# RuntimeRacer/vall-e

Hardware: AMD Instinct MI355X
Metric: AR codec-tokens/sec/GPU + NAR 7-stage p50 latency, d=1024 L=12 10s utterance (higher is better)
Workload: dtype bf16

## Files before the change

### vall-e_amd/csrc/ar_tp.hpp

```cpp
#pragma once
#include <type_traits>
#include "ar_granules.hpp"

namespace vx {

#ifdef VX_STAMPS
#define TP_STAMP(which, i)                                                                                            \
  do {                                                                                                                \
    unsigned long long* fq_r_ = g_fq_stamps;                                                                          \
    if (fq_r_ != nullptr && threadIdx.x == 0)                                                                         \
      fq_r_[(((size_t)(which) * 16 + a.layer) * 256 + blockIdx.x) * 16 + (i)] = __builtin_amdgcn_s_memrealtime();      \
  } while (0)
#else
#define TP_STAMP(which, i) do { } while (0)
#endif

constexpr int TP_D = 1024, TP_H = 16, TP_FF = 4096, TP_X = 8, TP_WG = 32;
constexpr int TP_HID = TP_FF / TP_X;
constexpr int TP_ACH = TP_D / TP_X;

struct TpAccArgs {
  long long* add;
  long long* zero;
  const float* bias;
};
constexpr float TP_FIX = 4294967296.0f, TP_UNFIX = 2.3283064365386963e-10f;
__device__ __forceinline__ long long tp_fix(float v) { return __float2ll_rn(v * TP_FIX); }

struct TpAttnArgs {
  const float* qkv_bias;
  unsigned* err;
  fq_gran* gq;
  fq_gran* gp;
  TpAccArgs acc;
  void* kcache;
  void* vcache;
  int ctx_max;
  float scale;
  int layer;
};

struct TpFfnArgs {
  const float* b1;
  unsigned* err;
  fq_gran* gh;
  TpAccArgs acc;
  int layer;
};

struct TpHeadArgs {
  float* logits;
  int N;
};

typedef float tp_f4 __attribute__((ext_vector_type(4)));
__device__ __forceinline__ void tp_ld16(vx_u32x4& v, const void* p) {
  asm volatile("global_load_dwordx4 %0, %1, off" : "=v"(v) : "v"(p) : "memory");
}
__device__ __forceinline__ void tp_ld16w(vx_u32x4& v, const void* p) {
  asm volatile("global_load_dwordx4 %0, %1, off" : "=v"(v) : "v"(p) : "memory");
}
__device__ __forceinline__ void tp_ld16f(tp_f4& v, const void* p) {
  asm volatile("global_load_dwordx4 %0, %1, off" : "=v"(v) : "v"(p) : "memory");
}
__device__ __forceinline__ void tp_ld4f(float& v, const void* p) {
  asm volatile("global_load_dword %0, %1, off" : "=v"(v) : "v"(p) : "memory");
}
template <int N> __device__ __forceinline__ void tp_wait() { asm volatile("s_waitcnt vmcnt(%0)" ::"n"(N) : "memory"); }
template <int N> __device__ __forceinline__ void tp_wait(vx_u32x4& a) { asm volatile("s_waitcnt vmcnt(%1)" : "+v"(a) : "n"(N) : "memory"); }
template <int N> __device__ __forceinline__ void tp_wait(float& a) { asm volatile("s_waitcnt vmcnt(%1)" : "+v"(a) : "n"(N) : "memory"); }
__device__ __forceinline__ uint4 tp_u4(const vx_u32x4& v) { return make_uint4(v.x, v.y, v.z, v.w); }

struct TpRowLoads { tp_f4 x, g, be; vx_u32x4 xf[2]; };
template <bool FIRST>
__device__ __forceinline__ void tp_row_issue(TpRowLoads& r, const float* __restrict__ x_f32, const long long* __restrict__ racc,
                                             const float* __restrict__ gbb, int tid) {
  if (FIRST) {
    tp_ld16f(r.x, x_f32 + 4 * tid);
  } else {
    tp_ld16(r.xf[0], racc + 4 * tid);
    tp_ld16(r.xf[1], racc + 4 * tid + 2);
  }
  tp_ld16f(r.g, gbb + 4 * tid);
  tp_ld16f(r.be, gbb + TP_D + 4 * tid);
}
template <bool FIRST, int AFTER> __device__ __forceinline__ void tp_row_wait(TpRowLoads& r) {
  if (FIRST) asm volatile("s_waitcnt vmcnt(%3)" : "+v"(r.x), "+v"(r.g), "+v"(r.be) : "n"(AFTER) : "memory");
  else asm volatile("s_waitcnt vmcnt(%4)" : "+v"(r.xf[0]), "+v"(r.xf[1]), "+v"(r.g), "+v"(r.be) : "n"(AFTER) : "memory");
}
__device__ __forceinline__ float tp_unfix(unsigned lo, unsigned hi) {
  return __ll2float_rn((long long)(((unsigned long long)hi << 32) | lo)) * TP_UNFIX;
}
template <typename WT> __device__ __forceinline__ float tp_exp(float v) {
  if constexpr (std::is_same<WT, float>::value) return expf(v);
  else return __expf(v);
}
template <bool FIRST>
__device__ __forceinline__ void tp_row_norm(TpRowLoads& r, float* xs, float* red, int tid) {
  const int lane = tid & 63, wave = tid >> 6;
  float4 v;
  if (FIRST) v = make_float4(r.x.x, r.x.y, r.x.z, r.x.w);
  else v = make_float4(tp_unfix(r.xf[0].x, r.xf[0].y), tp_unfix(r.xf[0].z, r.xf[0].w), tp_unfix(r.xf[1].x, r.xf[1].y), tp_unfix(r.xf[1].z, r.xf[1].w));
  float s1 = wave_sum_dpp((v.x + v.y) + (v.z + v.w));
  if (lane == 0) red[wave] = s1;
  __syncthreads();
  const float mean = ((red[0] + red[1]) + (red[2] + red[3])) * (1.0f / TP_D);
  const float d0 = v.x - mean, d1 = v.y - mean, d2 = v.z - mean, d3 = v.w - mean;
  float s2 = wave_sum_dpp((d0 * d0 + d1 * d1) + (d2 * d2 + d3 * d3));
  if (lane == 0) red[4 + wave] = s2;
  __syncthreads();
  const float rstd = 1.0f / sqrtf(((red[4] + red[5]) + (red[6] + red[7])) * (1.0f / TP_D) + LN_EPS);
  *reinterpret_cast<float4*>(xs + 4 * tid) =
      make_float4(d0 * rstd * r.g.x + r.be.x, d1 * rstd * r.g.y + r.be.y, d2 * rstd * r.g.z + r.be.z, d3 * rstd * r.g.w + r.be.w);
  __syncthreads();
}

template <bool FIRST>
__device__ __forceinline__ void tp_acc_add(const TpAccArgs& a, float partial, bool writer, int row, bool lead,
                                           unsigned long long carry_ll, float carry_f, float bo) {
  if (writer) {
    long long add = tp_fix(partial);
    if (lead) add += tp_fix(bo) + (FIRST ? tp_fix(carry_f) : (long long)carry_ll);
    atomicAdd(reinterpret_cast<unsigned long long*>(a.add) + row, (unsigned long long)add);
  }
}
__device__ __forceinline__ void tp_acc_zero(const TpAccArgs& a, bool zeroer, int tid) {
  if (zeroer) {
    *reinterpret_cast<uint4*>(a.zero + 4 * tid) = make_uint4(0u, 0u, 0u, 0u);
    *reinterpret_cast<uint4*>(a.zero + 4 * tid + 2) = make_uint4(0u, 0u, 0u, 0u);
  }
}
template <bool FIRST>
__device__ __forceinline__ void tp_acc_tail(const TpAccArgs& a, float partial, bool writer, int row, bool lead, int tid,
                                            unsigned long long carry_ll, float carry_f, float bo) {
  tp_acc_add<FIRST>(a, partial, writer, row, lead, carry_ll, carry_f, bo);
  tp_acc_zero(a, blockIdx.x == 1, tid);
}

template <int KCH, int VEC>
__device__ __forceinline__ void tp_row_read(const float* xs, int lane, float (&xr)[KCH][VEC]) {
#pragma unroll
  for (int c = 0; c < KCH; ++c)
#pragma unroll
    for (int i = 0; i < VEC; i += 4) {
      const float4 t = *reinterpret_cast<const float4*>(xs + (c * 64 + lane) * VEC + i);
      xr[c][i] = t.x; xr[c][i + 1] = t.y; xr[c][i + 2] = t.z; xr[c][i + 3] = t.w;
    }
}
template <typename WT, int KCH>
__device__ __forceinline__ float tp_dot(const uint4 (&w)[KCH], const float (&xr)[KCH][Vec16<WT>::N]) {
  constexpr int VEC = Vec16<WT>::N;
  float s = 0.f;
#pragma unroll
  for (int c = 0; c < KCH; ++c) {
    float wf[VEC];
    unpack<WT>(w[c], wf);
#pragma unroll
    for (int i = 0; i < VEC; ++i) s = fmaf(wf[i], xr[c][i], s);
  }
  return s;
}

template <int NGRP> struct TpAttnSmem {
  __attribute__((aligned(16))) float xs[TP_D];
  float red[8];
  __attribute__((aligned(16))) float s_qkv[FQ_QKV];
  __attribute__((aligned(16))) float sm_o[NGRP][64 + 4];
  float sm_m[4], sm_l[4];
  float s_wo[4][64];
  float s_part[FQ_S * FQ_PART];
  float s_fac[FQ_S];
  __attribute__((aligned(16))) float s_att[64];
};

template <typename WT, bool FIRST>
__device__ __forceinline__ void tp_attn_split(const void* __restrict__ Wqkv_, const float* __restrict__ x_f32,
                                              const long long* __restrict__ racc, const float* __restrict__ gbb,
                                              const ArState* __restrict__ st, const unsigned* __restrict__ epoch,
                                              const TpAttnArgs& a, TpAttnSmem<4 * Vec16<WT>::N>& sm) {
  constexpr int VEC = Vec16<WT>::N;
  constexpr int KCH = TP_D / (64 * VEC);
  constexpr int HD = 64;
  constexpr int LPK = HD / VEC, KPW = 64 / LPK, KPB = 4 * KPW, UNR = 4;
  float* const xs = sm.xs;
  float* const s_qkv = sm.s_qkv;
  const int tid = threadIdx.x, lane = tid & 63, wave = tid >> 6;
  const int x = blockIdx.x & (TP_X - 1), i = blockIdx.x >> 3;
  const int hl = i >> 4, j = i & 15, h = 2 * x + hl;
  const int cih = 8 * j + 2 * wave, ch = h * HD + cih;
  const int st_row = st->row;
  const unsigned tag = *epoch;
  const WT* __restrict__ W = reinterpret_cast<const WT*>(Wqkv_);

  TpRowLoads rl;
  tp_row_issue<FIRST>(rl, x_f32, racc, gbb, tid);
  TP_STAMP(0, 0);
  vx_u32x4 w[2][KCH];
#pragma unroll
  for (int r = 0; r < 2; ++r)
#pragma unroll
    for (int c = 0; c < KCH; ++c) tp_ld16w(w[r][c], W + (size_t)(ch + r) * TP_D + (c * 64 + lane) * VEC);
  float e_bias;
  {
    const float* bp = a.qkv_bias;
    asm volatile("" : "+s"(bp));
    tp_ld4f(e_bias, bp + ch + min(lane, 1));
  }
  const int n_old = st_row;
  const int chunk = (n_old + FQ_S - 1) / FQ_S;
  const int j0 = j * chunk, j1 = min(n_old, j0 + chunk);
  const int sub = lane % LPK, grp = lane / LPK;
  vx_u32x4 kr[UNR], vr[UNR];
  const WT* kb;
  const WT* vb;
  {
    const void* kcp = a.kcache;
    const void* vcp = a.vcache;
    int ctxm = a.ctx_max;
    asm volatile("" : "+s"(kcp), "+s"(vcp), "+s"(ctxm));
    kb = reinterpret_cast<const WT*>(kcp) + (size_t)h * ctxm * HD + sub * VEC;
    vb = reinterpret_cast<const WT*>(vcp) + (size_t)h * ctxm * HD + sub * VEC;
#pragma unroll
    for (int u = 0; u < UNR; ++u) {
      const int jk = min(j0 + u * KPB + wave * KPW + grp, max(j1, 1) - 1);
      tp_ld16(kr[u], kb + (size_t)jk * HD);
      tp_ld16(vr[u], vb + (size_t)jk * HD);
    }
  }
  auto load_pass = [&](int base) {
#pragma unroll
    for (int u = 0; u < UNR; ++u) {
      const int jk = min(base + u * KPB + wave * KPW + grp, max(j1, 1) - 1);
      const uint4 k4 = ld16(kb + (size_t)jk * HD), v4 = ld16(vb + (size_t)jk * HD);
      kr[u] = vx_u32x4{k4.x, k4.y, k4.z, k4.w};
      vr[u] = vx_u32x4{v4.x, v4.y, v4.z, v4.w};
    }
  };
  constexpr int N_KV = 2 * UNR, N_W = 2 * KCH;

  tp_row_wait<FIRST, N_W + 1 + N_KV>(rl);
  TP_STAMP(0, 7);
  tp_row_norm<FIRST>(rl, xs, sm.red, tid);
  TP_STAMP(0, 1);
  {
    float xr[KCH][VEC];
    tp_row_read<KCH, VEC>(xs, lane, xr);
    float acc[2];
#pragma unroll
    for (int r = 0; r < 2; ++r) {
      uint4 wr[KCH];
#pragma unroll
      for (int c = 0; c < KCH; ++c) { tp_wait<N_KV + 1>(w[r][c]); wr[c] = tp_u4(w[r][c]); }
      acc[r] = wave_sum_dpp(tp_dot<WT, KCH>(wr, xr));
    }
    tp_wait<N_KV>(e_bias);
    if (lane < 2) gran_store(a.gq + (size_t)h * FQ_QKV + cih + lane, (lane == 0 ? acc[0] : acc[1]) + e_bias, tag);
  }
  TP_STAMP(0, 2);
  const bool own_wg = (j == FQ_S - 1);
  {
    const int ng = own_wg ? FQ_QKV : HD;
    float v1[1];
    gran_gather<1>(a.gq + (size_t)h * FQ_QKV, ng, tag, v1, a.err, 1u);
    if (tid < ng) s_qkv[tid] = v1[0];
  }
#pragma unroll
  for (int u = 0; u < UNR; ++u) { tp_wait<0>(kr[u]); tp_wait<0>(vr[u]); }
  TP_STAMP(0, 3);
  __syncthreads();
  TP_STAMP(0, 8);
  float qv[VEC];
#pragma unroll
  for (int c = 0; c < VEC; ++c) qv[c] = s_qkv[sub * VEC + c] * a.scale;

  float M = -INFINITY, L = 0.f, acc[VEC];
#pragma unroll
  for (int c = 0; c < VEC; ++c) acc[c] = 0.f;
  const bool owner = own_wg && wave == 0;
  float sn = -INFINITY;
  if (owner) {
    float dot = 0.f;
#pragma unroll
    for (int c = 0; c < VEC; ++c) dot = fmaf(s_qkv[HD + sub * VEC + c], qv[c], dot);
    sn = (LPK == 8) ? group8_sum_dpp(dot) : group16_sum_dpp(dot);
  }
  for (int base = j0; base < j1 || (owner && base == j0); base += UNR * KPB) {
    if (base != j0) load_pass(base);
    const int nr = (j1 - base + KPB - 1) / KPB;
    float sc[UNR], mloc = (base == j0) ? sn : -INFINITY;
#pragma unroll
    for (int u = 0; u < UNR; ++u) {
      sc[u] = -INFINITY;
      if (u < nr) {
        const int jk = base + u * KPB + wave * KPW + grp;
        float kf[VEC];
        unpack<WT>(tp_u4(kr[u]), kf);
        float dot = 0.f;
#pragma unroll
        for (int c = 0; c < VEC; ++c) dot = fmaf(kf[c], qv[c], dot);
        dot = (LPK == 8) ? group8_sum_dpp(dot) : group16_sum_dpp(dot);
        sc[u] = (jk < j1) ? dot : -INFINITY;
        mloc = fmaxf(mloc, sc[u]);
      }
    }
    mloc = wave_max_dpp(mloc);
    if (mloc != -INFINITY) {
      const float Mn = fmaxf(M, mloc);
      const float corr = (M == -INFINITY) ? 0.f : tp_exp<WT>(M - Mn);
      L *= corr;
#pragma unroll
      for (int c = 0; c < VEC; ++c) acc[c] *= corr;
      M = Mn;
#pragma unroll
      for (int u = 0; u < UNR; ++u)
        if (u < nr) {
          float vf[VEC];
          unpack<WT>(tp_u4(vr[u]), vf);
          const float p = tp_exp<WT>(sc[u] - M);
          L += p;
#pragma unroll
          for (int c = 0; c < VEC; ++c) acc[c] = fmaf(p, vf[c], acc[c]);
        }
      if (owner && base == j0 && grp == 0) {
        const float p = tp_exp<WT>(sn - M);
        L += p;
#pragma unroll
        for (int c = 0; c < VEC; ++c) acc[c] = fmaf(p, s_qkv[2 * HD + sub * VEC + c], acc[c]);
      }
    }
  }
  TP_STAMP(0, 9);
  {
#pragma unroll
    for (int c = 0; c < VEC; c += 4)
      *reinterpret_cast<float4*>(&sm.sm_o[wave * KPW + grp][sub * VEC + c]) = make_float4(acc[c], acc[c + 1], acc[c + 2], acc[c + 3]);
    __builtin_amdgcn_fence(__ATOMIC_RELEASE, "wavefront");
    __builtin_amdgcn_wave_barrier();
    float oc = 0.f;
#pragma unroll
    for (int g = 0; g < KPW; ++g) oc += sm.sm_o[wave * KPW + g][lane];
    const float Lw = wave_sum_dpp(sub == 0 ? L : 0.f);
    sm.s_wo[wave][lane] = oc;
    if (lane == 0) { sm.sm_m[wave] = M; sm.sm_l[wave] = Lw; }
  }
  TP_STAMP(0, 10);
  __syncthreads();
  TP_STAMP(0, 11);
  if (tid < FQ_PART) {
    const float Mx = fmaxf(fmaxf(sm.sm_m[0], sm.sm_m[1]), fmaxf(sm.sm_m[2], sm.sm_m[3]));
    float v = 0.f;
    if (tid == HD) {
      v = Mx;
    } else {
#pragma unroll
      for (int wv = 0; wv < 4; ++wv)
        v = fmaf(tid < HD ? sm.s_wo[wv][tid] : sm.sm_l[wv], (sm.sm_m[wv] == -INFINITY) ? 0.f : tp_exp<WT>(sm.sm_m[wv] - Mx), v);
    }
    gran_store(a.gp + ((size_t)h * FQ_S + j) * FQ_PART + tid, v, tag);
  }
  TP_STAMP(0, 4);
  TP_STAMP(0, 5); TP_STAMP(0, 6);
}

template <typename WT, bool FIRST>
__device__ __forceinline__ void tp_attn_proj(const void* __restrict__ Wqkv_, const float* __restrict__ x_f32,
                                             const long long* __restrict__ racc, const float* __restrict__ gbb,
                                             const ArState* __restrict__ st, const unsigned* __restrict__ epoch,
                                             const void* __restrict__ Wo_, const TpAttnArgs& a,
                                             TpAttnSmem<4 * Vec16<WT>::N>& sm) {
  constexpr int VEC = Vec16<WT>::N;
  constexpr int KCH = TP_D / (64 * VEC);
  constexpr int HD = 64;
  constexpr int OCH = HD / (4 * VEC);
  float* const xs = sm.xs;
  const int tid = threadIdx.x, lane = tid & 63, wave = tid >> 6;
  const int x = blockIdx.x & (TP_X - 1), i = blockIdx.x >> 3;
  const int hl = i >> 4, jp = (i & 15) - FQ_S, h = 2 * x + hl;
  const int cih = 8 * jp + 2 * wave, ch = h * HD + cih;
  const int st_row = st->row, st_done = st->done;
  const unsigned tag = *epoch;
  const WT* __restrict__ W = reinterpret_cast<const WT*>(Wqkv_);

  TpRowLoads rl;
  tp_row_issue<FIRST>(rl, x_f32, racc, gbb, tid);
  TP_STAMP(0, 0);
  vx_u32x4 w[4][KCH];
#pragma unroll
  for (int r = 0; r < 4; ++r)
#pragma unroll
    for (int c = 0; c < KCH; ++c)
      tp_ld16w(w[r][c], W + (size_t)((1 + (r >> 1)) * TP_D + ch + (r & 1)) * TP_D + (c * 64 + lane) * VEC);
  float e_bias;
  {
    const float* bp = a.qkv_bias;
    asm volatile("" : "+s"(bp));
    const int r = min(lane, 3);
    tp_ld4f(e_bias, bp + (1 + (r >> 1)) * TP_D + ch + (r & 1));
  }
  const int orow = 128 * jp + (tid >> 2);
  unsigned long long carry_ll[2] = {0ull, 0ull};
  float carry_f[2] = {0.f, 0.f}, bo[2];
#pragma unroll
  for (int s = 0; s < 2; ++s) {
    if (FIRST) tp_ld4f(carry_f[s], x_f32 + orow + 64 * s);
    else asm volatile("global_load_dwordx2 %0, %1, off" : "=v"(carry_ll[s]) : "v"(racc + orow + 64 * s) : "memory");
    tp_ld4f(bo[s], a.acc.bias + orow + 64 * s);
  }
  vx_u32x4 wo[2][OCH];
  {
    const uint4* wb = reinterpret_cast<const uint4*>(Wo_) + (size_t)(x * TP_WG + 16 * hl + 2 * jp) * OCH * 256;
#pragma unroll
    for (int s = 0; s < 2; ++s)
#pragma unroll
      for (int m = 0; m < OCH; ++m) tp_ld16w(wo[s][m], wb + (s * OCH + m) * 256 + tid);
  }
  constexpr int N_WO = 2 * OCH, N_W = 4 * KCH;

  tp_row_wait<FIRST, N_W + 5 + N_WO>(rl);
  TP_STAMP(0, 7);
  tp_row_norm<FIRST>(rl, xs, sm.red, tid);
  TP_STAMP(0, 1);
  {
    float xr[KCH][VEC];
    tp_row_read<KCH, VEC>(xs, lane, xr);
    float acc[4];
#pragma unroll
    for (int r = 0; r < 4; ++r) {
      uint4 wr[KCH];
#pragma unroll
      for (int c = 0; c < KCH; ++c) { tp_wait<N_WO + 5>(w[r][c]); wr[c] = tp_u4(w[r][c]); }
      acc[r] = wave_sum_dpp(tp_dot<WT, KCH>(wr, xr));
    }
    tp_wait<N_WO + 4>(e_bias);
    if (lane < 4) {
      const int kv = lane >> 1, c = cih + (lane & 1);
      const WT rv = from_f32<WT>((lane == 0 ? acc[0] : lane == 1 ? acc[1] : lane == 2 ? acc[2] : acc[3]) + e_bias);
      if (!st_done) {
        WT* cache = reinterpret_cast<WT*>(kv == 0 ? a.kcache : a.vcache);
        cache[((size_t)h * a.ctx_max + st_row) * HD + c] = rv;
      }
      gran_store(a.gq + (size_t)h * FQ_QKV + (1 + kv) * HD + c, to_f32(rv), tag);
    }
  }
  TP_STAMP(0, 2);
  TP_STAMP(0, 3); TP_STAMP(0, 8); TP_STAMP(0, 9); TP_STAMP(0, 10); TP_STAMP(0, 11); TP_STAMP(0, 4);
  {
    constexpr int NG = (FQ_S * FQ_PART + 255) / 256;
    float pv[NG];
    gran_gather<NG>(a.gp + (size_t)h * FQ_S * FQ_PART, FQ_S * FQ_PART, tag, pv, a.err, 2u);
#pragma unroll
    for (int g = 0; g < NG; ++g)
      if (tid + 256 * g < FQ_S * FQ_PART) sm.s_part[tid + 256 * g] = pv[g];
  }
#pragma unroll
  for (int s = 0; s < 2; ++s) {
#pragma unroll
    for (int m = 0; m < OCH; ++m) tp_wait<0>(wo[s][m]);
    asm volatile("" : "+v"(carry_ll[s]), "+v"(carry_f[s]), "+v"(bo[s]));
  }
  TP_STAMP(0, 5);
  __syncthreads();
  if (tid < FQ_S) {
    const float* hp = sm.s_part;
    float Mx = hp[HD];
#pragma unroll
    for (int s = 1; s < FQ_S; ++s) Mx = fmaxf(Mx, hp[s * FQ_PART + HD]);
    const float pm = hp[tid * FQ_PART + HD];
    const float es = (pm == -INFINITY) ? 0.f : tp_exp<WT>(pm - Mx);
    const float Ls = group8_sum_dpp(hp[tid * FQ_PART + HD + 1] * es);
    sm.s_fac[tid] = es * (1.0f / Ls);
  }
  __syncthreads();
  if (tid < HD) {
    float o = 0.f;
#pragma unroll
    for (int s = 0; s < FQ_S; ++s) o = fmaf(sm.s_part[s * FQ_PART + tid], sm.s_fac[s], o);
    sm.s_att[tid] = o;
  }
  __syncthreads();
#pragma unroll
  for (int sl = 0; sl < 2; ++sl) {
    float s = 0.f;
#pragma unroll
    for (int m = 0; m < OCH; ++m) {
      float wf[VEC];
      unpack<WT>(tp_u4(wo[sl][m]), wf);
      const float* ap = sm.s_att + ((tid & 3) + 4 * m) * VEC;
#pragma unroll
      for (int c = 0; c < VEC; ++c) s = fmaf(wf[c], ap[c], s);
    }
    s = group4_sum_dpp(s);
    tp_acc_add<FIRST>(a.acc, s, (tid & 3) == 0, orow + 64 * sl, h == 0, carry_ll[sl], carry_f[sl], bo[sl]);
  }
  tp_acc_zero(a.acc, blockIdx.x == TP_X * FQ_S + 1, tid);
  TP_STAMP(0, 6);
}

template <typename WT, bool FIRST>
__global__ __launch_bounds__(256) void tp_attn_kernel(const void* __restrict__ Wqkv_, const float* __restrict__ x_f32,
                                                      const long long* __restrict__ racc, const float* __restrict__ gbb,
                                                      const ArState* __restrict__ st, const unsigned* __restrict__ epoch,
                                                      const void* __restrict__ Wo_, const TpAttnArgs a) {
  __shared__ TpAttnSmem<4 * Vec16<WT>::N> sm;
  if (((blockIdx.x >> 3) & (FQ_G - 1)) < FQ_S) tp_attn_split<WT, FIRST>(Wqkv_, x_f32, racc, gbb, st, epoch, a, sm);
  else tp_attn_proj<WT, FIRST>(Wqkv_, x_f32, racc, gbb, st, epoch, Wo_, a, sm);
}

template <typename WT>
__global__ __launch_bounds__(256) void tp_ffn_kernel(const void* __restrict__ W1_, const long long* __restrict__ racc,
                                                     const float* __restrict__ gbb,
                                                     const unsigned* __restrict__ epoch, const void* __restrict__ W2_,
                                                     const TpFfnArgs a) {
  constexpr int VEC = Vec16<WT>::N;
  constexpr int KCH = TP_D / (64 * VEC);
  constexpr int FCH = TP_HID / (8 * VEC);
  __shared__ __attribute__((aligned(16))) float xs[TP_D];
  __shared__ float red[8];
  __shared__ __attribute__((aligned(16))) float hs[TP_HID];
  const int tid = threadIdx.x, lane = tid & 63, wave = tid >> 6;
  const int x = blockIdx.x & (TP_X - 1), i = blockIdx.x >> 3;
  const unsigned tag = *epoch;
  const WT* __restrict__ W1 = reinterpret_cast<const WT*>(W1_);
  const int row0 = TP_HID * x + 16 * i + 4 * wave;

  TpRowLoads rl;
  tp_row_issue<false>(rl, nullptr, racc, gbb, tid);
  TP_STAMP(1, 0);
  vx_u32x4 w1[4][KCH];
#pragma unroll
  for (int r = 0; r < 4; ++r)
#pragma unroll
    for (int c = 0; c < KCH; ++c) tp_ld16w(w1[r][c], W1 + (size_t)(row0 + r) * TP_D + (c * 64 + lane) * VEC);
  float e_b1;
  {
    const float* bp = a.b1;
    asm volatile("" : "+s"(bp));
    tp_ld4f(e_b1, bp + row0 + min(lane, 3));
  }
  unsigned long long carry_ll;
  float bo;
  asm volatile("global_load_dwordx2 %0, %1, off" : "=v"(carry_ll) : "v"(racc + 32 * i + (tid >> 3)) : "memory");
  tp_ld4f(bo, a.acc.bias + 32 * i + (tid >> 3));
  vx_u32x4 w2[FCH];
  auto tp_stage2 = [&]() {
    const uint4* wb = reinterpret_cast<const uint4*>(W2_) + (size_t)(x * TP_WG + i) * FCH * 256;
#pragma unroll
    for (int m = 0; m < FCH; ++m) tp_ld16w(w2[m], wb + m * 256 + tid);
  };
  tp_stage2();
  tp_row_wait<false, 4 * KCH + 3 + FCH>(rl);
  TP_STAMP(1, 7);
  tp_row_norm<false>(rl, xs, red, tid);
  TP_STAMP(1, 1);
  {
    float xr[KCH][VEC];
    tp_row_read<KCH, VEC>(xs, lane, xr);
    float acc[4];
#pragma unroll
    for (int r = 0; r < 4; ++r) {
      uint4 wr[KCH];
#pragma unroll
      for (int c = 0; c < KCH; ++c) { tp_wait<3 + FCH>(w1[r][c]); wr[c] = tp_u4(w1[r][c]); }
      acc[r] = wave_sum_dpp(tp_dot<WT, KCH>(wr, xr));
    }
    tp_wait<2 + FCH>(e_b1);
    if (lane < 4) {
      const float v = (lane == 0 ? acc[0] : lane == 1 ? acc[1] : lane == 2 ? acc[2] : acc[3]) + e_b1;
      gran_store(a.gh + (size_t)x * TP_HID + 16 * i + 4 * wave + lane, fmaxf(v, 0.f), tag);
    }
  }
  TP_STAMP(1, 2);
  {
    float hv[2];
    gran_gather<2>(a.gh + (size_t)x * TP_HID, TP_HID, tag, hv, a.err, 3u);
    hs[tid] = hv[0]; hs[tid + 256] = hv[1];
  }
#pragma unroll
  for (int m = 0; m < FCH; ++m) tp_wait<0>(w2[m]);
  asm volatile("" : "+v"(carry_ll), "+v"(bo));
  TP_STAMP(1, 3);
  __syncthreads();
  {
    float s = 0.f;
#pragma unroll
    for (int m = 0; m < FCH; ++m) {
      float wf[VEC];
      unpack<WT>(tp_u4(w2[m]), wf);
      const float* hp = hs + ((tid & 7) + 8 * m) * VEC;
#pragma unroll
      for (int c = 0; c < VEC; ++c) s = fmaf(wf[c], hp[c], s);
    }
    s = group8_sum_dpp(s);
    tp_acc_tail<false>(a.acc, s, (tid & 7) == 0, 32 * i + (tid >> 3), x == 0, tid, carry_ll, 0.f, bo);
  }
  TP_STAMP(1, 4);
}

template <typename WT>
__global__ __launch_bounds__(256) void tp_head_kernel(const void* __restrict__ W_, const long long* __restrict__ racc,
                                                      const float* __restrict__ gbb,
                                                      const ArState* __restrict__ st, const TpHeadArgs a) {
  constexpr int VEC = Vec16<WT>::N;
  constexpr int KCH = TP_D / (64 * VEC);
  __shared__ __attribute__((aligned(16))) float xs[TP_D];
  __shared__ float red[8];
  const int tid = threadIdx.x, lane = tid & 63, wave = tid >> 6;
  const WT* __restrict__ W = reinterpret_cast<const WT*>(W_);
  const int row0 = (blockIdx.x * 4 + wave) * 4;
  TpRowLoads rl;
  tp_row_issue<false>(rl, nullptr, racc, gbb, tid);
  vx_u32x4 w[4][KCH];
#pragma unroll
  for (int r = 0; r < 4; ++r)
#pragma unroll
    for (int c = 0; c < KCH; ++c) tp_ld16w(w[r][c], W + (size_t)min(row0 + r, a.N - 1) * TP_D + (c * 64 + lane) * VEC);
  const int st_pass = st->pass, st_trace = st->trace_logits, st_done = st->done;
  tp_row_wait<false, 4 * KCH>(rl);
  tp_row_norm<false>(rl, xs, red, tid);
  float xr[KCH][VEC];
  tp_row_read<KCH, VEC>(xs, lane, xr);
  float acc[4];
#pragma unroll
  for (int r = 0; r < 4; ++r) {
    uint4 wr[KCH];
#pragma unroll
    for (int c = 0; c < KCH; ++c) { tp_wait<0>(w[r][c]); wr[c] = tp_u4(w[r][c]); }
    acc[r] = wave_sum_dpp(tp_dot<WT, KCH>(wr, xr));
  }
  const int row = row0 + lane;
  if (lane < 4 && row < a.N && !st_done) {
    const float v = lane == 0 ? acc[0] : lane == 1 ? acc[1] : lane == 2 ? acc[2] : acc[3];
    a.logits[row] = v;
    if (st_trace) a.logits[LOGITS_CUR + (size_t)st_pass * a.N + row] = v;
  }
}

template <typename WT, bool HEADS>
__global__ void tp_repack_kernel(const WT* __restrict__ src, uint4* __restrict__ dst, int K) {
  constexpr int VEC = Vec16<WT>::N;
  const int KX = K / TP_X, NW = KX / (8 * VEC);
  const size_t word = (size_t)blockIdx.x * 256 + threadIdx.x;
  const size_t total = (size_t)TP_D * K / VEC;
  if (word >= total) return;
  const int t = (int)(word & 255);
  const size_t blk = word >> 8;
  const int m = (int)(blk % NW);
  const int wg = (int)(blk / NW);
  const int x = wg / TP_WG, i = wg % TP_WG;
  int row, col;
  if (HEADS) {
    row = 64 * (i & 15) + (t >> 2);
    col = 64 * (2 * x + (i >> 4)) + ((t & 3) + 4 * m) * VEC;
  } else {
    row = 32 * i + (t >> 3);
    col = KX * x + ((t & 7) + 8 * m) * VEC;
  }
  dst[word] = *reinterpret_cast<const uint4*>(src + (size_t)row * K + col);
}

}
```

Measured before the change: 5124.

## Move current-token attention score from split workgroup into the output-projection merge stage

The split-attention stage no longer has one designated workgroup per head that waits for the full new q/k/v row and folds the current token's score and value into its partial softmax. Instead, the merge/output-projection stage gathers the new q/k/v, computes the self-score there, and adds it as an extra term in the cross-split softmax combine. This removes the extra wait and imbalance on the owner workgroup in the attention pass. In exchange it adds a gather and a barrier to the merge stage, which now has to wait for the freshly written K/V before it can finish.

New measurement: 5148, median of 2. Within noise of the previous version (+0.5%).

```diff
diff --git a/vall-e_amd/csrc/ar_tp.hpp b/vall-e_amd/csrc/ar_tp.hpp
--- a/vall-e_amd/csrc/ar_tp.hpp
+++ b/vall-e_amd/csrc/ar_tp.hpp
@@ -169,7 +169,7 @@
   float sm_m[4], sm_l[4];
   float s_wo[4][64];
   float s_part[FQ_S * FQ_PART];
-  float s_fac[FQ_S];
+  float s_fac[FQ_S + 1];
   __attribute__((aligned(16))) float s_att[64];
 };
 
@@ -257,12 +257,10 @@
     if (lane < 2) gran_store(a.gq + (size_t)h * FQ_QKV + cih + lane, (lane == 0 ? acc[0] : acc[1]) + e_bias, tag);
   }
   TP_STAMP(0, 2);
-  const bool own_wg = (j == FQ_S - 1);
-  {
-    const int ng = own_wg ? FQ_QKV : HD;
+  {
     float v1[1];
-    gran_gather<1>(a.gq + (size_t)h * FQ_QKV, ng, tag, v1, a.err, 1u);
-    if (tid < ng) s_qkv[tid] = v1[0];
+    gran_gather<1>(a.gq + (size_t)h * FQ_QKV, HD, tag, v1, a.err, 1u);
+    if (tid < HD) s_qkv[tid] = v1[0];
   }
 #pragma unroll
   for (int u = 0; u < UNR; ++u) { tp_wait<0>(kr[u]); tp_wait<0>(vr[u]); }
@@ -276,18 +274,10 @@
   float M = -INFINITY, L = 0.f, acc[VEC];
 #pragma unroll
   for (int c = 0; c < VEC; ++c) acc[c] = 0.f;
-  const bool owner = own_wg && wave == 0;
-  float sn = -INFINITY;
-  if (owner) {
-    float dot = 0.f;
-#pragma unroll
-    for (int c = 0; c < VEC; ++c) dot = fmaf(s_qkv[HD + sub * VEC + c], qv[c], dot);
-    sn = (LPK == 8) ? group8_sum_dpp(dot) : group16_sum_dpp(dot);
-  }
-  for (int base = j0; base < j1 || (owner && base == j0); base += UNR * KPB) {
+  for (int base = j0; base < j1; base += UNR * KPB) {
     if (base != j0) load_pass(base);
     const int nr = (j1 - base + KPB - 1) / KPB;
-    float sc[UNR], mloc = (base == j0) ? sn : -INFINITY;
+    float sc[UNR], mloc = -INFINITY;
 #pragma unroll
     for (int u = 0; u < UNR; ++u) {
       sc[u] = -INFINITY;
@@ -321,12 +311,6 @@
 #pragma unroll
           for (int c = 0; c < VEC; ++c) acc[c] = fmaf(p, vf[c], acc[c]);
         }
-      if (owner && base == j0 && grp == 0) {
-        const float p = tp_exp<WT>(sn - M);
-        L += p;
-#pragma unroll
-        for (int c = 0; c < VEC; ++c) acc[c] = fmaf(p, s_qkv[2 * HD + sub * VEC + c], acc[c]);
-      }
     }
   }
   TP_STAMP(0, 9);
@@ -443,7 +427,29 @@
     }
   }
   TP_STAMP(0, 2);
-  TP_STAMP(0, 3); TP_STAMP(0, 8); TP_STAMP(0, 9); TP_STAMP(0, 10); TP_STAMP(0, 11); TP_STAMP(0, 4);
+  {
+    float v1[1];
+    gran_gather<1>(a.gq + (size_t)h * FQ_QKV, FQ_QKV, tag, v1, a.err, 4u);
+    if (tid < FQ_QKV) sm.s_qkv[tid] = v1[0];
+  }
+#pragma unroll
+  for (int s = 0; s < 2; ++s) {
+#pragma unroll
+    for (int m = 0; m < OCH; ++m) tp_wait<0>(wo[s][m]);
+    asm volatile("" : "+v"(carry_ll[s]), "+v"(carry_f[s]), "+v"(bo[s]));
+  }
+  TP_STAMP(0, 3);
+  __syncthreads();
+  float sn;
+  {
+    constexpr int LPK = HD / VEC;
+    const int sub = lane % LPK;
+    float dot = 0.f;
+#pragma unroll
+    for (int c = 0; c < VEC; ++c) dot = fmaf(sm.s_qkv[HD + sub * VEC + c], sm.s_qkv[sub * VEC + c] * a.scale, dot);
+    sn = (LPK == 8) ? group8_sum_dpp(dot) : group16_sum_dpp(dot);
+  }
+  TP_STAMP(0, 8); TP_STAMP(0, 9); TP_STAMP(0, 10); TP_STAMP(0, 11); TP_STAMP(0, 4);
   {
     constexpr int NG = (FQ_S * FQ_PART + 255) / 256;
     float pv[NG];
@@ -452,30 +458,26 @@
     for (int g = 0; g < NG; ++g)
       if (tid + 256 * g < FQ_S * FQ_PART) sm.s_part[tid + 256 * g] = pv[g];
   }
-#pragma unroll
-  for (int s = 0; s < 2; ++s) {
-#pragma unroll
-    for (int m = 0; m < OCH; ++m) tp_wait<0>(wo[s][m]);
-    asm volatile("" : "+v"(carry_ll[s]), "+v"(carry_f[s]), "+v"(bo[s]));
-  }
   TP_STAMP(0, 5);
   __syncthreads();
   if (tid < FQ_S) {
     const float* hp = sm.s_part;
-    float Mx = hp[HD];
-#pragma unroll
-    for (int s = 1; s < FQ_S; ++s) Mx = fmaxf(Mx, hp[s * FQ_PART + HD]);
+    float Mx = sn;
+#pragma unroll
+    for (int s = 0; s < FQ_S; ++s) Mx = fmaxf(Mx, hp[s * FQ_PART + HD]);
     const float pm = hp[tid * FQ_PART + HD];
     const float es = (pm == -INFINITY) ? 0.f : tp_exp<WT>(pm - Mx);
-    const float Ls = group8_sum_dpp(hp[tid * FQ_PART + HD + 1] * es);
-    sm.s_fac[tid] = es * (1.0f / Ls);
+    const float en = tp_exp<WT>(sn - Mx);
+    const float rL = 1.0f / (group8_sum_dpp(hp[tid * FQ_PART + HD + 1] * es) + en);
+    sm.s_fac[tid] = es * rL;
+    if (tid == 0) sm.s_fac[FQ_S] = en * rL;
   }
   __syncthreads();
   if (tid < HD) {
     float o = 0.f;
 #pragma unroll
     for (int s = 0; s < FQ_S; ++s) o = fmaf(sm.s_part[s * FQ_PART + tid], sm.s_fac[s], o);
-    sm.s_att[tid] = o;
+    sm.s_att[tid] = fmaf(sm.s_qkv[2 * HD + tid], sm.s_fac[FQ_S], o);
   }
   __syncthreads();
 #pragma unroll
```
